# MaxInGaussian/SCFGP

Hardware: AMD Instinct MI355X
Metric: NLML+grad evals/sec (higher is better)
Workload: dtype f32

## Files before the change

### scfgp_amd/csrc/apply.hip

```cpp
#include "kernels.h"
#include "tile_cfgs.h"

#include <algorithm>

#ifdef SCFGP_TRACE
constexpr int ATRACE_CAP = 1 << 16;
__device__ unsigned long long g_atrace[5 * ATRACE_CAP][5];
int64_t apply_trace_read(void* host, int64_t max_bytes) {
    const int64_t n = max_bytes < (int64_t)sizeof(g_atrace) ? max_bytes : (int64_t)sizeof(g_atrace);
    return hipMemcpyFromSymbol(host, HIP_SYMBOL(g_atrace), n) == hipSuccess ? n : -2;
}
#else
int64_t apply_trace_read(void*, int64_t) { return -1; }
#endif
template <typename T, int TILE> struct ApplyCfg {
    typedef TileCfg<T, Tune<T>::APPLY_BM, TILE, SCFGP_BK, Tune<T>::APPLY_WGM, Tune<T>::apply_wgn(TILE), Tune<T>::MS,
                    SCFGP_BK == 16 && Tune<T>::MS == 16> type;
};

#include "apply_epilogue.h"

template <class Cfg, int EPI>
__device__ __forceinline__ void apply_tile(
    const typename Cfg::T* __restrict__ Phi, const typename Cfg::T* __restrict__ Bm, typename Cfg::T* V,
// ... 22 lines not shown
    if constexpr (EPI != 1 && EPI != 4) { if (want_mu) la.dot_reduce(mu + (int64_t)(jt0 + jt) * Np + rb * Cfg::BM); }
    apply_epilogue<Cfg, EPI>(acc, Phi, V, vpart, p, q, y, alpha, ut, K, Kp, Np, rb, cbase, jt0 + jt, smem_raw);
}

template <class Cfg, int EPI>
__global__ __launch_bounds__(Cfg::THREADS) __attribute__((amdgpu_waves_per_eu(1, 8)))
void apply_kernel(
    const typename Cfg::T* __restrict__ Phi, const typename Cfg::T* __restrict__ Bm, typename Cfg::T* V,
    double* __restrict__ vpart, const double* __restrict__ p, const double* __restrict__ q, const double* __restrict__ y,
    const double* __restrict__ alpha, const double* __restrict__ ut, int K, int Kp, int64_t Np, int njt,
    int col0, int jt0, double* __restrict__ mu, int ntot) {
    SMEM_DECL;
    const unsigned wid = xcd_remap(blockIdx.x, gridDim.x);
    if constexpr (EPI == 3 || EPI == 4) {
        const int np = (njt + 1) / 2, t = (int)(wid % np), o = njt - 1 - t;
        const int64_t rb = wid / np;
        apply_tile<Cfg, EPI>(Phi, Bm, V, vpart, p, q, y, alpha, ut, K, Kp, Np, njt, col0, jt0, mu, ntot, t, rb, smem_raw);
        if (o != t) {
            __syncthreads();
            apply_tile<Cfg, EPI>(Phi, Bm, V, vpart, p, q, y, alpha, ut, K, Kp, Np, njt, col0, jt0, mu, ntot, o, rb, smem_raw);
        }
    } else
        apply_tile<Cfg, EPI>(Phi, Bm, V, vpart, p, q, y, alpha, ut, K, Kp, Np, njt, col0, jt0, mu, ntot, (int)(wid % njt), wid / njt, smem_raw);
}

typedef __attribute__((address_space(3))) void lds_void;
typedef const __attribute__((address_space(1))) void gbl_void;
template <typename T, int BN_>
struct ApplyDma {
    static constexpr int ES = (int)sizeof(T), BM = 256, BN = BN_, ROWB = 16 * ES, CPR = ROWB / 16;
    static constexpr int WN = ES == 4 ? 64 : 32;
    static constexpr int WAVES = 4 * (BN / WN), STAGE = (BM + BN) * ROWB, STAGES = 3, LDS_BYTES = STAGES * STAGE,
                         DMA_PER_WAVE = STAGE / 1024 / WAVES, ROWS_PER_DMA = 1024 / ROWB;
    static constexpr int PRE = 2;
    static constexpr int WAVES_PER_EU = WAVES == 4 ? 2 : 4;
    typedef TileCfg<T, BM, BN, 16, 4, BN / WN, 16, true> Cfg;
    static_assert(STAGE / 1024 % WAVES == 0 && LDS_BYTES <= 160 * 1024, "whole DMA instructions per wave; the ring fits the LDS");
    static __device__ __forceinline__ int swz(int x) {
        if constexpr (ES == 4) return (0x78 >> (2 * ((x >> 2) & 3))) & 3;
        else return (int)((0x6BEB08u >> (3 * ((x >> 1) & 7))) & 7);
    }
};
static_assert(((0x6BEB08u >> 0) & 7) == 0 && ((0x6BEB08u >> 3) & 7) == 1 && ((0x6BEB08u >> 6) & 7) == 4 && ((0x6BEB08u >> 9) & 7) == 5 &&
              ((0x6BEB08u >> 12) & 7) == 6 && ((0x6BEB08u >> 15) & 7) == 7 && ((0x6BEB08u >> 18) & 7) == 2 && ((0x6BEB08u >> 21) & 7) == 3,
              "fp64 swizzle table");

template <typename T, int EPI, int BN>
__global__ __launch_bounds__((64 * ApplyDma<T, BN>::WAVES)) __attribute__((amdgpu_waves_per_eu(ApplyDma<T, BN>::WAVES_PER_EU, ApplyDma<T, BN>::WAVES_PER_EU)))
void apply_dma_kernel(const T* __restrict__ Phi, const T* __restrict__ Bm, T* V,
                      double* __restrict__ vpart, const double* __restrict__ p, const double* __restrict__ q,
                      const double* __restrict__ y, const double* __restrict__ alpha, const double* __restrict__ ut,
                      int K, int Kp, int64_t Np, int njt, double* __restrict__ mu, int col0, int slot0, int64_t rb0) {
    typedef ApplyDma<T, BN> D;
    typedef typename D::Cfg Cfg;
    typedef T half_t __attribute__((ext_vector_type(2)));
    typedef std::integral_constant<int, 0> H0;
    typedef std::integral_constant<int, 1> H1;
    constexpr int DPW = D::DMA_PER_WAVE, NRD = Cfg::TM + Cfg::TN, NM = 2 * Cfg::TM * Cfg::TN, PRE = D::PRE;
    static_assert(Cfg::TM == 4 && (Cfg::TN == 4 || Cfg::TN == 2), "fragment lists of the wait statements");
    static_assert(PRE + DPW + NRD <= NM, "one fetch or read per MFMA behind the barrier");
    SMEM_DECL;
    char* smem = smem_raw;
#ifdef SCFGP_TRACE
    const unsigned long long tr_t0 = __builtin_amdgcn_s_memrealtime();
#endif
    const unsigned wid = xcd_remap(blockIdx.x, gridDim.x);
    const int jt = EPI == 3 || EPI == 4 ? (int)((wid % njt + wid / njt) % njt) : (int)(wid % njt);
    const int64_t rb = rb0 + wid / njt;
    const int cbase = col0 + jt * D::BN;
    const int lane = threadIdx.x & 63, wave = __builtin_amdgcn_readfirstlane(threadIdx.x >> 6);
    const char* src[DPW]; unsigned loff[DPW]; int dst[DPW];
#pragma unroll
    for (int u = 0; u < DPW; ++u) {
        const int t = wave * DPW + u, x0 = D::ROWS_PER_DMA * t, l = lane / D::CPR, c = (lane % D::CPR) ^ D::swz(x0 + l);
        const int xb = x0 - D::BM, xcol = (xb & ~(D::WN - 1)) + Cfg::TN * (xb & 15) + ((xb >> 4) & (Cfg::TN - 1));
        const T* rowp = x0 < D::BM ? Phi + (rb * D::BM + x0) * Kp : Bm + (int64_t)(cbase + xcol) * Kp;
        src[u] = reinterpret_cast<const char*>(rowp) + (EPI == 4 ? (cbase / 16) * D::ROWB : 0);
        loff[u] = (unsigned)((x0 < D::BM ? l : Cfg::TN * l) * Kp * D::ES + c * 16);
        dst[u] = t * 1024;
    }
    const auto fetch_one = [&](auto uc, int slot) {
        constexpr int u = decltype(uc)::value;
        __builtin_amdgcn_global_load_lds((gbl_void*)(src[u] + loff[u]), (lds_void*)(smem + slot * D::STAGE + dst[u]), 16, 0, 0);
        src[u] += D::ROWB;
    };
    const int i = lane & 15, qg = lane >> 4;
    const int wm0 = (wave / Cfg::WGN) * Cfg::WM, wn0 = (wave % Cfg::WGN) * Cfg::WN;
    const int hoff0 = sizeof(T) == 4 ? (((qg >> 1) ^ D::swz(i)) << 4) + 8 * (qg & 1) : ((2 * qg) ^ D::swz(i)) << 4;
    const int hoff1 = sizeof(T) == 4 ? (((2 + (qg >> 1)) ^ D::swz(i)) << 4) + 8 * (qg & 1) : ((2 * qg + 1) ^ D::swz(i)) << 4;
    const int ring = (int)(uintptr_t)smem, aoff = ring + (wm0 + i) * D::ROWB, boff = ring + D::BM * D::ROWB + (wn0 + i) * D::ROWB;
    const int ra[2] = {aoff + hoff0, aoff + hoff1}, rbb[2] = {boff + hoff0, boff + hoff1};
    half_t ha[2][Cfg::TM], hb[2][Cfg::TN];
    typename Cfg::MTr::acc_t acc[Cfg::TM][Cfg::TN];
    acc_zero<Cfg>(acc);
    const int nst_all = (K + 15) / 16, nst_tri = (cbase + D::BN + 15) / 16;
    const int nst = (EPI == 3 && nst_tri < nst_all ? nst_tri : nst_all) - (EPI == 4 ? cbase / 16 : 0);
#define SCFGP_LDS_READ(dst, addr, off)                                                                              \
    do {                                                                                                             \
        if constexpr (sizeof(T) == 4) asm volatile("ds_read_b64 %0, %1 offset:%2" : "=v"(dst) : "v"(addr), "n"(off));   \
        else asm volatile("ds_read_b128 %0, %1 offset:%2" : "=v"(dst) : "v"(addr), "n"(off));                           \
    } while (0)
    const auto read_one = [&](auto hc, auto rc, int stage) {
// ... 5 lines not shown
#define SCFGP_WAIT_FRAGS(what, h)                                                                                                   \
    do {                                                                                                                            \
        if constexpr (Cfg::TN == 4)                                                                                                 \
            asm volatile("s_waitcnt " what : "+v"(ha[h][0]), "+v"(ha[h][1]), "+v"(ha[h][2]), "+v"(ha[h][3]),                        \
                                             "+v"(hb[h][0]), "+v"(hb[h][1]), "+v"(hb[h][2]), "+v"(hb[h][3]) :: "memory");           \
        else                                                                                                                        \
            asm volatile("s_waitcnt " what : "+v"(ha[h][0]), "+v"(ha[h][1]), "+v"(ha[h][2]), "+v"(ha[h][3]),                        \
                                             "+v"(hb[h][0]), "+v"(hb[h][1]) :: "memory");                                           \
    } while (0)
    const auto mfma_one = [&](auto hc, auto ic) {
        constexpr int h = decltype(hc)::value, I = decltype(ic)::value, j = I / (Cfg::TM * Cfg::TN), tm = I / Cfg::TN % Cfg::TM, tn = I % Cfg::TN;
        Cfg::MTr::mfma(acc[tm][tn], ha[h][tm][j], hb[h][tn][j]);
        __builtin_amdgcn_sched_barrier(0);
    };
    const auto second_half_pre = [&]() { static_for<PRE>([&](auto ic) { mfma_one(H1(), ic); }); };
    const auto second_half = [&](auto fc, int fslot, int next) {
        static_for<NM - PRE>([&](auto ic) {
            constexpr int I = decltype(ic)::value;
            mfma_one(H1(), std::integral_constant<int, I + PRE>());
            if constexpr (I < DPW) {
                if constexpr (decltype(fc)::value) { fetch_one(ic, fslot); __builtin_amdgcn_sched_barrier(0); }
            } else if constexpr (I - DPW < NRD) {
                read_one(H0(), std::integral_constant<int, I - DPW>(), next);
                __builtin_amdgcn_sched_barrier(0);
            }
        });
    };
    const auto first_half = [&](int next) {
        static_for<NM>([&](auto ic) {
            mfma_one(H0(), ic);
            if constexpr (decltype(ic)::value < NRD) { read_one(H1(), ic, next); __builtin_amdgcn_sched_barrier(0); }
        });
    };
    static_for<DPW>([&](auto uc) { fetch_one(uc, 0); });
    if (nst > 1) static_for<DPW>([&](auto uc) { fetch_one(uc, 1); });
    if (nst > 2) static_for<DPW>([&](auto uc) { fetch_one(uc, 2); });
    if (nst > 2) asm volatile("s_waitcnt vmcnt(%0)" :: "n"(2 * DPW) : "memory");
    else if (nst > 1) asm volatile("s_waitcnt vmcnt(%0)" :: "n"(DPW) : "memory");
    else asm volatile("s_waitcnt vmcnt(0)" ::: "memory");
    __builtin_amdgcn_s_barrier();
    asm volatile("" ::: "memory");
#ifdef SCFGP_TRACE
    const unsigned long long tr_l0 = __builtin_amdgcn_s_memrealtime();
#endif
    static_for<NRD>([&](auto rc) { read_one(H0(), rc, 0); });
    static_for<NRD>([&](auto rc) { read_one(H1(), rc, 0); });
    SCFGP_WAIT_FRAGS("lgkmcnt(0)", 0);
    __builtin_amdgcn_sched_barrier(0);
    static_for<NM>([&](auto ic) { mfma_one(H0(), ic); });
    int slot = 0, s = 0;
    for (; s + 3 < nst; ++s) {
        asm volatile("s_waitcnt vmcnt(%0)" :: "n"(DPW) : "memory");
        SCFGP_WAIT_FRAGS("lgkmcnt(0)", 1);
        __builtin_amdgcn_sched_barrier(0);
        second_half_pre();
        __builtin_amdgcn_s_barrier();
        asm volatile("" ::: "memory");
        const int fslot = slot;
        slot = slot == 2 ? 0 : slot + 1;
        __builtin_amdgcn_sched_barrier(0);
        second_half(std::true_type(), fslot, slot * D::STAGE);
        SCFGP_WAIT_FRAGS("lgkmcnt(0)", 0);
        __builtin_amdgcn_sched_barrier(0);
        first_half(slot * D::STAGE);
    }
    SCFGP_WAIT_FRAGS("lgkmcnt(0)", 1);
    for (; s + 1 < nst; ++s) {
        if (s + 2 < nst) asm volatile("s_waitcnt vmcnt(%0)" :: "n"(DPW) : "memory");
        else asm volatile("s_waitcnt vmcnt(0)" ::: "memory");
        SCFGP_WAIT_FRAGS("lgkmcnt(0)", 1);
        __builtin_amdgcn_sched_barrier(0);
        second_half_pre();
        __builtin_amdgcn_s_barrier();
        asm volatile("" ::: "memory");
        slot = slot == 2 ? 0 : slot + 1;
        __builtin_amdgcn_sched_barrier(0);
        second_half(std::false_type(), 0, slot * D::STAGE);
        SCFGP_WAIT_FRAGS("lgkmcnt(0)", 0);
        __builtin_amdgcn_sched_barrier(0);
        first_half(slot * D::STAGE);
    }
    SCFGP_WAIT_FRAGS("lgkmcnt(0)", 1);
    __builtin_amdgcn_sched_barrier(0);
    static_for<NM>([&](auto ic) { mfma_one(H1(), ic); });
#undef SCFGP_WAIT_FRAGS
    __syncthreads();
#ifdef SCFGP_TRACE
    const unsigned long long tr_l1 = __builtin_amdgcn_s_memrealtime();
#endif
    constexpr int SLOTS = BN >= 128 ? BN / 128 : 1;
    const int vslot = slot0 + SLOTS * jt;
    int tid = (int)threadIdx.x;
    asm volatile("" : "+v"(tid));
    apply_epilogue<Cfg, EPI, EPI == 0 || EPI == 3, true>(acc, Phi, V, vpart, p, q, y, alpha, ut, K, Kp, Np, rb, cbase, vslot, smem_raw, mu, tid);
    if (SLOTS == 2 && (EPI == 0 || EPI == 3) && tid < D::BM) {
        vpart[(int64_t)(vslot + 1) * Np + rb * D::BM + tid] = 0.0;
        if (mu) mu[(int64_t)(vslot + 1) * Np + rb * D::BM + tid] = 0.0;
    }
#ifdef SCFGP_TRACE
    __syncthreads();
    if (threadIdx.x == 0 && blockIdx.x < ATRACE_CAP) {
        unsigned long long* rec = g_atrace[EPI * ATRACE_CAP + blockIdx.x];
        rec[0] = tr_t0; rec[1] = __builtin_amdgcn_s_memrealtime();
        rec[2] = ((unsigned long long)__builtin_amdgcn_s_getreg((20 << 0) | (0 << 6) | (3 << 11)) & 0xF) | ((unsigned long long)jt << 8) |
                                  ((unsigned long long)nst << 20);
        rec[3] = tr_l0; rec[4] = tr_l1;
    }
#endif
}

template <typename T> struct ApplyPlan {
    static constexpr int NW = 2;
    int width[NW], count[NW], col0[NW], jt0[NW], total;
    explicit ApplyPlan(int K) {
        const int w[NW] = {128, 64};
        int col = 0, jt = 0;
        const bool small = K <= 256;
        for (int i = 0; i < NW; ++i) {
            width[i] = w[i];
            const bool last = i == NW - 1;
            count[i] = small && !last ? 0 : (last ? (K - col + w[i] - 1) / w[i] : (K - col) / w[i]);
            col0[i] = col; jt0[i] = jt;
            col += count[i] * w[i]; jt += count[i];
        }
        total = jt;
    }
};
bool F16x3Kernels::apply_runs(const Geom& g) { return ApplyPlan<float>(g.K).count[0] > 0; }
template <class Cfg, int EPI, typename T>
static int apply_launch_cfg(const Geom& g, int njt, int col0, int jt0, const T* Phi, const T* Bm, T* V, double* vpart,
                            const double* p, const double* q, const double* y, const double* alpha, const double* ut,
                            double* mu, int ntot, hipStream_t st) {
    if (njt <= 0) return 0;
    const int64_t nrb = g.Np / Cfg::BM;
    const int wgs_per_rb = EPI == 3 || EPI == 4 ? (njt + 1) / 2 : njt;
    allow_big_lds(apply_kernel<Cfg, EPI>, Cfg::LDS_BYTES);
    hipLaunchKernelGGL((apply_kernel<Cfg, EPI>), dim3((unsigned)(wgs_per_rb * nrb)), dim3(Cfg::THREADS), Cfg::LDS_BYTES, st,
                       Phi, Bm, V, vpart, p, q, y, alpha, ut, g.K, g.Kp, g.Np, njt, col0, jt0, mu, ntot);
    return (int)(njt * nrb);
}
template <typename T, int EPI, int BN>
static int apply_dma_launch(const Geom& g, int njt, int col0, int slot0, const T* Phi, const T* Bm, T* V, double* vpart,
                            const double* p, const double* q, const double* y, const double* alpha, const double* ut,
                            double* mu, hipStream_t st, int64_t rb0 = 0, int64_t nrb = -1) {
    typedef ApplyDma<T, BN> D;
    if (nrb < 0) nrb = g.Np / D::BM;
    if (njt <= 0 || nrb <= 0) return 0;
    allow_big_lds(apply_dma_kernel<T, EPI, BN>, D::LDS_BYTES);
    hipLaunchKernelGGL((apply_dma_kernel<T, EPI, BN>), dim3((unsigned)(njt * nrb)), dim3(64 * D::WAVES), D::LDS_BYTES, st,
                       Phi, Bm, V, vpart, p, q, y, alpha, ut, g.K, g.Kp, g.Np, njt, mu, col0, slot0, rb0);
    return (int)(njt * nrb);
}
static int apply_num_cus() {
    static int n = 0;
    if (n == 0) {
        int dev = 0; hipDeviceProp_t prop;
        if (hipGetDevice(&dev) == hipSuccess && hipGetDeviceProperties(&prop, dev) == hipSuccess) n = prop.multiProcessorCount;
        if (n <= 0) n = 256;
    }
    return n;
}
template <typename T, int EPI>
static int apply_launch(const Geom& g, const T* Phi, const T* Bm, T* V, double* vpart, const double* p, const double* q,
                        const double* y, const double* alpha, const double* ut, double* mu, hipStream_t st,
                        int dma = 0, const T* BmT = nullptr, const F16Operands* f16 = nullptr) {
    if (!BmT) BmT = Bm;
    const ApplyPlan<T> pl(g.K);
    int nb = 0;
    if constexpr (EPI != 2) {
        if (dma && pl.count[0] > 0) {
            int n256 = 0;
            const int64_t nrb = g.Np / 256;
            int64_t tail_rb = 0;
            if constexpr (sizeof(T) == 4) {
                n256 = dma == 2 ? pl.count[0] / 2 : 0;
                if (n256 > 0 && EPI != 3 && EPI != 4) {
                    const int64_t ncu = apply_num_cus(), tiles = nrb * n256, rem = tiles % ncu;
                    if (tiles > ncu && rem > 0 && 20 * rem <= 9 * ncu) tail_rb = (rem + n256 - 1) / n256;
                }
                if (f16 && (EPI == 0 || EPI == 1)) {
                    constexpr int E = EPI == 1 ? 1 : 0;
                    nb += F16x3Kernels::apply<E, 256>(g, n256, 0, 0, Phi, *f16, V, vpart, p, q, y, alpha, ut, mu, st, 0, nrb - tail_rb);
                    nb += F16x3Kernels::apply<E, 128>(g, pl.count[0] - 2 * n256, 256 * n256, 2 * n256, Phi, *f16, V, vpart, p, q, y, alpha, ut, mu, st, 0, nrb - tail_rb);
                    nb += F16x3Kernels::apply<E, 64>(g, pl.count[1], pl.col0[1], pl.jt0[1], Phi, *f16, V, vpart, p, q, y, alpha, ut, mu, st, 0, nrb - tail_rb);
                    if (tail_rb > 0) {
                        nb += F16x3Kernels::apply<E, 128>(g, pl.count[0], 0, 0, Phi, *f16, V, vpart, p, q, y, alpha, ut, mu, st, nrb - tail_rb, tail_rb);
                        nb += F16x3Kernels::apply<E, 64>(g, pl.count[1], pl.col0[1], pl.jt0[1], Phi, *f16, V, vpart, p, q, y, alpha, ut, mu, st, nrb - tail_rb, tail_rb);
                    }
                    return nb;
                }
                nb += apply_dma_launch<T, EPI, 256>(g, n256, 0, 0, Phi, BmT, V, vpart, p, q, y, alpha, ut, mu, st, 0, nrb - tail_rb);
            }
            nb += apply_dma_launch<T, EPI, 128>(g, pl.count[0] - 2 * n256, 256 * n256, 2 * n256, Phi, BmT, V, vpart, p, q, y, alpha, ut, mu, st, 0, nrb - tail_rb);
            nb += apply_dma_launch<T, EPI, 64>(g, pl.count[1], pl.col0[1], pl.jt0[1], Phi, BmT, V, vpart, p, q, y, alpha, ut, mu, st, 0, nrb - tail_rb);
            if (tail_rb > 0) {
                nb += apply_dma_launch<T, EPI, 128>(g, pl.count[0], 0, 0, Phi, BmT, V, vpart, p, q, y, alpha, ut, mu, st, nrb - tail_rb, tail_rb);
                nb += apply_dma_launch<T, EPI, 64>(g, pl.count[1], pl.col0[1], pl.jt0[1], Phi, BmT, V, vpart, p, q, y, alpha, ut, mu, st, nrb - tail_rb, tail_rb);
            }
            return nb;
        }
    }
    nb += apply_launch_cfg<typename ApplyCfg<T, 128>::type, EPI, T>(g, pl.count[0], pl.col0[0], pl.jt0[0], Phi, Bm, V, vpart, p, q, y, alpha, ut, mu, pl.total, st);
    nb += apply_launch_cfg<typename ApplyCfg<T, 64>::type, EPI, T>(g, pl.count[1], pl.col0[1], pl.jt0[1], Phi, Bm, V, vpart, p, q, y, alpha, ut, mu, pl.total, st);
    return nb;
}

template <typename T>
void ApplyKernels<T>::apply_v(const Geom& g, const T* Phi, const T* Bm, T* V, double* vpart, const double* alpha, double* mu,
                              hipStream_t st, int dma, const F16Operands* f16) {
    apply_launch<T, 0>(g, Phi, Bm, V, vpart, nullptr, nullptr, nullptr, alpha, nullptr, mu, st, dma, nullptr, f16);
}
template <typename T>
void ApplyKernels<T>::apply_predict(const Geom& g, const T* Phi, const T* LiT, double* vpart, const double* alpha, double* mu,
                                    hipStream_t st) {
    apply_launch<T, 2>(g, Phi, LiT, (T*)nullptr, vpart, nullptr, nullptr, nullptr, alpha, nullptr, mu, st);
}
template <typename T>
void ApplyKernels<T>::apply_plain(const Geom& g, const T* A, const T* Bm, T* Out, int Kc, int ncols, hipStream_t st) {
    Geom gk = g; gk.K = Kc;
    apply_launch_cfg<typename ApplyCfg<T, 64>::type, 4, T>(gk, (ncols + 63) / 64, 0, 0, A, Bm, Out, nullptr, nullptr, nullptr, nullptr, nullptr,
                                                           nullptr, nullptr, ApplyPlan<T>(Kc).total, st);
}

template <typename T>
void ApplyKernels<T>::apply_c(const Geom& g, const T* Phi, const T* LiT, const T* Li, T* C, double* vpart, const double* alpha,
                              const double* beta, double* mu, hipStream_t st, int dma) {
    const bool by_dma = dma && ApplyPlan<T>(g.K).count[0] > 0;
    apply_launch<T, 3>(g, Phi, LiT, C, vpart, nullptr, nullptr, nullptr, by_dma ? beta : alpha, nullptr, mu, st, dma, Li);
}
template <typename T>
void ApplyKernels<T>::apply_vc(const Geom& g, const T* C, const T* Li, const T* LiT, T* V, hipStream_t st, int dma) {
    apply_launch<T, 4>(g, C, Li, V, nullptr, nullptr, nullptr, nullptr, nullptr, nullptr, nullptr, st, dma, LiT);
}
template <typename T>
void ApplyKernels<T>::apply_phibar(const Geom& g, const T* Phi, const T* Abar, T* V, const double* p, const double* q,
                                   const double* y, const double* alpha, const double* ut, hipStream_t st, int dma, const F16Operands* f16) {
    apply_launch<T, 1>(g, Phi, Abar, V, nullptr, p, q, y, alpha, ut, nullptr, st, dma, nullptr, f16);
}

template <typename T> static int apply_njt(const Geom& g) { return ApplyPlan<T>(g.K).total; }


template <int MODE>
__global__ __launch_bounds__(256) void rowstats_kernel(const double* __restrict__ mupart, const double* __restrict__ vpart, int njt,
                                                       const double* __restrict__ y, const Scal* __restrict__ sc,
                                                       double* __restrict__ o1, double* __restrict__ o2,
                                                       double* __restrict__ partial, int64_t N, int64_t Np) {
    __shared__ double red[4][256];
    const double kappa = sc->kappa;
    double t2 = 0, kb = 0, qv = 0, pm = 0;
    for (int64_t n = (int64_t)blockIdx.x * 256 + threadIdx.x; n < Np; n += (int64_t)gridDim.x * 256) {
        double v = 0, mu = 0;
        for (int t = 0; t < njt; ++t) { v += vpart[(int64_t)t * Np + n]; mu += mupart[(int64_t)t * Np + n]; }
        const double d = kappa * (v + 1.0);
        if (MODE == 0) {
            double pn = 0, qn = 0;
            if (n < N) {
                const double r = mu - y[n];
                const double rv = r * r + v;
                const double e = 1.0 / d - rv / (d * d);
                pn = 2.0 * r / d;
                qn = 1.0 / d + kappa * e;
                t2 += rv / d + log(2.0 * M_PI * d);
                kb += e * (v + 1.0);
                qv += qn * v; pm += pn * mu;
            }
            o1[n] = pn; o2[n] = qn;
        } else if (n < N) {
            o1[n] = mu; o2[n] = sqrt(d);
        }
    }
    if (MODE == 0) {
        red[0][threadIdx.x] = t2; red[1][threadIdx.x] = kb; red[2][threadIdx.x] = qv; red[3][threadIdx.x] = pm;
        __syncthreads();
        for (int w = 128; w >= 1; w >>= 1) {
            if ((int)threadIdx.x < w)
                for (int k = 0; k < 4; ++k) red[k][threadIdx.x] += red[k][threadIdx.x + w];
            __syncthreads();
        }
        if (threadIdx.x < 4) partial[blockIdx.x * 4 + threadIdx.x] = red[threadIdx.x][0];
    }
}

template <typename T>
void ApplyKernels<T>::rowstats(const Geom& g, const double* mupart, const double* vpart, const double* y,
                               const Scal* sc, double* p, double* q, double* partial, int nblocks, hipStream_t st) {
    hipLaunchKernelGGL((rowstats_kernel<0>), dim3(nblocks), dim3(256), 0, st, mupart, vpart, apply_njt<T>(g), y, sc, p, q,
                       partial, g.N, g.Np);
}

template <typename T>
void ApplyKernels<T>::rowpredict(const Geom& g, const double* mupart, const double* vpart, const Scal* sc, double* mu, double* sd,
                                 hipStream_t st) {
    const int nblocks = (int)((g.Np + 255) / 256 < 1024 ? (g.Np + 255) / 256 : 1024);
    hipLaunchKernelGGL((rowstats_kernel<1>), dim3(nblocks), dim3(256), 0, st, mupart, vpart, apply_njt<T>(g),
                       (const double*)nullptr, sc, mu, sd, (double*)nullptr, g.N, g.Np);
}
template <typename T> int ApplyKernels<T>::partials(const Geom& g) { return apply_njt<T>(g); }
__global__ __launch_bounds__(256) void rowresidual_kernel(const double* __restrict__ mupart, int njt, const double* __restrict__ y,
                                                          double* __restrict__ r, int64_t N, int64_t Np) {
    for (int64_t n = (int64_t)blockIdx.x * 256 + threadIdx.x; n < Np; n += (int64_t)gridDim.x * 256) {
        double mu = 0;
        for (int t = 0; t < njt; ++t) mu += mupart[(int64_t)t * Np + n];
        r[n] = n < N ? y[n] - mu : 0.0;
    }
}
template <typename T>
void ApplyKernels<T>::rowresidual(const Geom& g, const double* mupart, const double* y, double* r, hipStream_t st) {
    const int nblocks = (int)((g.Np + 255) / 256 < 1024 ? (g.Np + 255) / 256 : 1024);
    hipLaunchKernelGGL(rowresidual_kernel, dim3(nblocks), dim3(256), 0, st, mupart, apply_njt<T>(g), y, r, g.N, g.Np);
}
template struct ApplyKernels<double>;
template struct ApplyKernels<float>;

__global__ __launch_bounds__(256) void reduce_scalars_kernel(const double* __restrict__ partial, int nblocks, int width,
                                                             double* __restrict__ scalars, int slot0) {
    __shared__ double red[256];
    for (int k = 0; k < width; ++k) {
        double s = 0;
        for (int b = threadIdx.x; b < nblocks; b += 256) s += partial[(int64_t)b * width + k];
        red[threadIdx.x] = s;
        __syncthreads();
        for (int m = 128; m >= 1; m >>= 1) {
            if (threadIdx.x < m) red[threadIdx.x] += red[threadIdx.x + m];
            __syncthreads();
        }
        if (threadIdx.x == 0) scalars[slot0 + k] = red[0];
        __syncthreads();
    }
// ... 54 lines not shown
```

### scfgp_amd/csrc/apply_epilogue.h

```cpp
#pragma once
#include "kernels.h"
#include "tile_cfgs.h"

template <int CTRL> __device__ __forceinline__ double dpp_mov_f64(double x) {
    int lo = __double2loint(x), hi = __double2hiint(x);
    lo = __builtin_amdgcn_update_dpp(0, lo, CTRL, 0xF, 0xF, true);
    hi = __builtin_amdgcn_update_dpp(0, hi, CTRL, 0xF, 0xF, true);
    return __hiloint2double(hi, lo);
}
__device__ __forceinline__ double row16_sum(double x) {
    x += dpp_mov_f64<0xB1>(x);
    x += dpp_mov_f64<0x4E>(x);
    x += dpp_mov_f64<0x141>(x);
    x += dpp_mov_f64<0x140>(x);
    return x;
}
template <class Cfg, int EPI, bool MU>
__device__ __forceinline__ void apply_epilogue_vec2(
    const typename Cfg::MTr::acc_t (&acc)[Cfg::TM][Cfg::TN], const double* __restrict__ Phi, double* V,
    double* __restrict__ vpart, const double* __restrict__ p, const double* __restrict__ q, const double* __restrict__ y,
    const double* __restrict__ alpha, const double* __restrict__ ut, int K, int Kp, int64_t Np, int64_t rb, int cbase, int jtg,
    char* smem_raw, double* __restrict__ mupart, int tid) {
    static_assert(Cfg::TN == 2 && Cfg::MS == 16 && sizeof(typename Cfg::T) == 8 && (EPI == 0 || EPI == 1 || EPI == 3 || EPI == 4), "VEC2 layout");
    AccCoord<Cfg> co(tid);
// ... 46 lines not shown
            if (MU && mupart) mupart[(int64_t)jtg * Np + rb * Cfg::BM + tid] = s2;
        }
    } else {
        double al[2], u2[2];
#pragma unroll
        for (int k = 0; k < 2; ++k) { al[k] = alpha[jg + k]; u2[k] = ut[jg + k]; }
        double* rowsc = reinterpret_cast<double*>(smem_raw);
        for (int i = tid; i < Cfg::BM; i += Cfg::THREADS) {
            const int64_t n = rb * Cfg::BM + i;
            rowsc[3 * i] = 2.0 * q[n]; rowsc[3 * i + 1] = p[n]; rowsc[3 * i + 2] = y[n];
        }
        __syncthreads();
#pragma unroll
        for (int tm = 0; tm < Cfg::TM; ++tm) {
            v2d vv[4];
            int64_t off[4];
#pragma unroll
            for (int r = 0; r < 4; ++r) {
                off[r] = (rb * Cfg::BM + co.row(tm, r)) * Kp + jg;
                vv[r] = *reinterpret_cast<const v2d*>(V + off[r]);
            }
#pragma unroll
            for (int r = 0; r < 4; ++r) {
                const int row = co.row(tm, r);
                const double qn = rowsc[3 * row], pn = rowsc[3 * row + 1], yn = rowsc[3 * row + 2];
                v2d o;
#pragma unroll
                for (int k = 0; k < 2; ++k) o[k] = 2.0 * acc[tm][k][r] + qn * vv[r][k] + pn * al[k] + yn * u2[k];
                *reinterpret_cast<v2d*>(V + off[r]) = o;
            }
        }
    }
}
template <class Cfg, int EPI, bool MU = false, bool VEC4 = false>
__device__ __forceinline__ void apply_epilogue(
    const typename Cfg::MTr::acc_t (&acc)[Cfg::TM][Cfg::TN], const typename Cfg::T* __restrict__ Phi, typename Cfg::T* V,
    double* __restrict__ vpart, const double* __restrict__ p, const double* __restrict__ q, const double* __restrict__ y,
    const double* __restrict__ alpha, const double* __restrict__ ut, int K, int Kp, int64_t Np, int64_t rb, int cbase, int jtg,
    char* smem_raw, double* __restrict__ mupart = nullptr, int tid = (int)threadIdx.x) {
    typedef typename Cfg::T T;
    if constexpr (VEC4 && sizeof(T) == 8) {
        apply_epilogue_vec2<Cfg, EPI, MU>(acc, Phi, V, vpart, p, q, y, alpha, ut, K, Kp, Np, rb, cbase, jtg, smem_raw, mupart, tid);
        return;
    }
    AccCoord<Cfg> co(tid);
    if constexpr (VEC4 && sizeof(T) == 4) {
        static_assert(Cfg::TN == 4 && Cfg::MS == 16 && sizeof(T) == 4 && (EPI == 0 || EPI == 1 || EPI == 3 || EPI == 4), "VEC4 layout");
        const int c4 = co.wn0 + 4 * (co.lane & 15);
        const int jg = cbase + c4;
        if constexpr (EPI == 4) {
#pragma unroll
            for (int tm = 0; tm < Cfg::TM; ++tm)
#pragma unroll
                for (int r = 0; r < 4; ++r)
                    *reinterpret_cast<v4f*>(V + (rb * Cfg::BM + co.row(tm, r)) * Kp + jg) = v4f{acc[tm][0][r], acc[tm][1][r], acc[tm][2][r], acc[tm][3][r]};
        } else if constexpr (EPI == 0 || EPI == 3) {
            double* red = reinterpret_cast<double*>(smem_raw);
            double* red2 = red + Cfg::WGN * Cfg::BM;
            const int wn = (tid >> 6) % Cfg::WGN;
            double al[4], live[4];
#pragma unroll
            for (int k = 0; k < 4; ++k) { live[k] = jg + k < K ? 1.0 : 0.0; al[k] = MU && jg + k < K ? alpha[jg + k] : 0.0; }
#pragma unroll
            for (int tm = 0; tm < Cfg::TM; ++tm) {
                v4f ph[4];
                int64_t off[4];
#pragma unroll
                for (int r = 0; r < 4; ++r) {
                    off[r] = (rb * Cfg::BM + co.row(tm, r)) * Kp + jg;
                    if (EPI == 0) ph[r] = *reinterpret_cast<const v4f*>(Phi + off[r]);
                }
#pragma unroll
                for (int r = 0; r < 4; ++r) {
                    const int row = co.row(tm, r);
                    const v4f c = v4f{acc[tm][0][r], acc[tm][1][r], acc[tm][2][r], acc[tm][3][r]};
                    *reinterpret_cast<v4f*>(V + off[r]) = c;
                    double part = 0, mup = 0;
                    if (EPI == 3) {
                        part = (double)(c[0] * c[0]) + (double)(c[1] * c[1]) + (double)(c[2] * c[2]) + (double)(c[3] * c[3]);
                        if (MU) mup = (double)c[0] * al[0] + (double)c[1] * al[1] + (double)c[2] * al[2] + (double)c[3] * al[3];
                    } else {
#pragma unroll
                        for (int k = 0; k < 4; ++k) { part += (double)ph[r][k] * (double)c[k] * live[k]; if (MU) mup += (double)ph[r][k] * al[k]; }
                    }
                    part = row16_sum(part);
                    if ((co.lane & 15) == 0) red[wn * Cfg::BM + row] = part;
                    if (MU) {
                        mup = row16_sum(mup);
                        if ((co.lane & 15) == 0) red2[wn * Cfg::BM + row] = mup;
                    }
                }
            }
            __syncthreads();
            if (tid < Cfg::BM) {
                double s = 0, s2 = 0;
#pragma unroll
                for (int k = 0; k < Cfg::WGN; ++k) { s += red[k * Cfg::BM + tid]; if (MU) s2 += red2[k * Cfg::BM + tid]; }
                vpart[(int64_t)jtg * Np + rb * Cfg::BM + tid] = s;
                if (MU && mupart) mupart[(int64_t)jtg * Np + rb * Cfg::BM + tid] = s2;
            }
        } else {
            float alf[4], u4f[4];
#pragma unroll
            for (int k = 0; k < 4; ++k) { alf[k] = (float)alpha[jg + k]; u4f[k] = (float)ut[jg + k]; }
            float* rowsc = reinterpret_cast<float*>(smem_raw);
            for (int i = tid; i < Cfg::BM; i += Cfg::THREADS) {
                const int64_t n = rb * Cfg::BM + i;
                rowsc[3 * i] = (float)(2.0 * q[n]); rowsc[3 * i + 1] = (float)p[n]; rowsc[3 * i + 2] = (float)y[n];
            }
            __syncthreads();
#pragma unroll
            for (int tm = 0; tm < Cfg::TM; ++tm) {
                v4f vv[4];
                int64_t off[4];
#pragma unroll
                for (int r = 0; r < 4; ++r) {
                    off[r] = (rb * Cfg::BM + co.row(tm, r)) * Kp + jg;
                    vv[r] = *reinterpret_cast<const v4f*>(V + off[r]);
                }
#pragma unroll
                for (int r = 0; r < 4; ++r) {
                    const int row = co.row(tm, r);
                    const float qn = rowsc[3 * row], pn = rowsc[3 * row + 1], yn = rowsc[3 * row + 2];
                    v4f o;
#pragma unroll
                    for (int k = 0; k < 4; ++k) o[k] = fmaf(qn, vv[r][k], fmaf(pn, alf[k], fmaf(yn, u4f[k], 2.0f * acc[tm][k][r])));
                    *reinterpret_cast<v4f*>(V + off[r]) = o;
                }
            }
        }
        return;
    }
    if (EPI == 4) {
// ... 89 lines not shown
```

### scfgp_amd/csrc/kernels.h

```cpp
#pragma once
#include "common.h"

struct Geom {
    int D, S, M, J, K, P;
    int Dp;
    int Jp;
    int Sp;
    int lowrank;
    int Kp;
    int tile;
    int gfull;
    int gstrip;
    int64_t N;
    int64_t Np;
};

struct RowSplits {
    int nsplit;
    int groups;
    int units;
    int taper;
    int gran;
    int64_t nrb;
    __host__ __device__ int per_group() const { return units + taper; }
// ... 22 lines not shown
    static void featuremap(const Geom& g, const double* Xt, const Projection& pr, const Scal* sc, T* Phi, hipStream_t st);
    static void convert(const double* src, T* dst, int K, int Kp, hipStream_t st);
    static void convert_transposed(const double* src, T* dst, int K, int Kp, hipStream_t st);
};

template <typename T>
struct GramKernels {
    static void gram(const Geom& g, const T* Phi, const double* w, const double* side, const RowSplits& rs, int64_t chunk,
                     double* slabs, double* sidepart, int* qhead, float* ws2, hipStream_t st);
    static int gram_jobs(const Geom& g);
    static void xtz(const Geom& g, const double* Xt, const T* Phi, const T* Phibar, int nsplit, int64_t chunk, double* slabs,
                    hipStream_t st);
    static void zbar_inplace(const Geom& g, const T* Phi, T* Phibar, hipStream_t st);
    static void rsel(const Geom& g, const double* params, T* out, hipStream_t st);
    static void tn_plain(const double* A, int Dp, const T* Bm, int64_t ldb, int J, int64_t Np, int nsplit, int64_t chunk, double* slabs,
                         hipStream_t st);
};

struct F16Operands { const unsigned* Phi16; const char* B16; const float* scale; unsigned* V16; const float* vbound; };

template <typename T>
struct ApplyKernels {
    static void apply_v(const Geom& g, const T* Phi, const T* Bm, T* V, double* vpart, const double* alpha, double* mupart,
                        hipStream_t st, int dma = 0, const F16Operands* f16 = nullptr);
    static void apply_predict(const Geom& g, const T* Phi, const T* LiT, double* vpart, const double* alpha, double* mupart,
                              hipStream_t st);
    static void apply_c(const Geom& g, const T* Phi, const T* LiT, const T* Li, T* C, double* vpart, const double* alpha,
                        const double* beta, double* mupart, hipStream_t st, int dma = 0);
    static void apply_vc(const Geom& g, const T* C, const T* Li, const T* LiT, T* V, hipStream_t st, int dma = 0);
    static void apply_phibar(const Geom& g, const T* Phi, const T* Abar, T* V, const double* p, const double* q,
                             const double* y, const double* alpha, const double* ut, hipStream_t st, int dma = 0, const F16Operands* f16 = nullptr);
    static void apply_plain(const Geom& g, const T* A, const T* Bm, T* Out, int Kc, int ncols, hipStream_t st);
    static void rowstats(const Geom& g, const double* mupart, const double* vpart, const double* y,
                         const Scal* sc, double* p, double* q, double* partial, int nblocks, hipStream_t st);
    static void rowpredict(const Geom& g, const double* mupart, const double* vpart, const Scal* sc, double* mu, double* sd,
                           hipStream_t st);
    static void rowresidual(const Geom& g, const double* mupart, const double* y, double* r, hipStream_t st);
    static int partials(const Geom& g);
};

struct F16x3Kernels {
    static void split_operand(const Geom& g, const double* M, char* B16, float* scale, double* part, const Scal* sc, hipStream_t st);
    template <int EPI, int BN>
    static int apply(const Geom& g, int njt, int col0, int slot0, const float* Phi, const F16Operands& f, float* V,
                     double* vpart, const double* p, const double* q, const double* y, const double* alpha, const double* ut, double* mu,
                     hipStream_t st, int64_t rb0, int64_t nrb);
    static bool apply_runs(const Geom& g);
    static constexpr size_t F16_PAD = 1024;
    static int side_blocks(const Geom& g);
    static void split_phi(const Geom& g, const float* Phi, const double* y, const Scal* sc, unsigned* Phi16, double* sidepart, float* tmp,
                          hipStream_t st);
    static void v_bound(const Geom& g, const double* B, const Scal* sc, float* tmp, hipStream_t st);
    static void split_v(const Geom& g, const float* V, const double* q, const double* p, unsigned* V16g, unsigned* qV16g, double* sidepart,
                        float* tmp, hipStream_t st);
    static int gram_chunks(const Geom& g, int64_t chunk);
    static int gram_tiles(const Geom& g);
    static void gram(const Geom& g, const unsigned* A16g, const unsigned* B16g, const float* scale, int64_t chunk, double* slabs, hipStream_t st);
};

template <typename T> struct SweepKernels : FmapKernels<T>, GramKernels<T>, ApplyKernels<T> {};

int64_t trace_read(void* host, int64_t max_bytes);
int64_t apply_trace_read(void* host, int64_t max_bytes);
int64_t chol_trace_read(void* host, int64_t max_bytes);

void reduce_tri_tiles(const double* slabs, int nsplit, int nts, int tile, double* packed, hipStream_t st);
void unpack_tri_tiles(const double* packed, int nts, int tile, double* full, int64_t ld, hipStream_t st);
// ... 145 lines not shown
```

### scfgp_amd/csrc/scfgp_api.hip

```cpp
#include "../../include/scfgp_hip.h"
#include "kernels.h"

#include <dlfcn.h>
#if __has_include(<rccl/rccl.h>)
#include <rccl/rccl.h>
#else
extern "C" {
typedef struct ncclComm* ncclComm_t;
typedef struct { char internal[128]; } ncclUniqueId;
typedef enum { ncclSuccess = 0 } ncclResult_t;
typedef enum { ncclFloat64 = 8 } ncclDataType_t;
typedef enum { ncclSum = 0 } ncclRedOp_t;
ncclResult_t ncclGetUniqueId(ncclUniqueId*);
ncclResult_t ncclCommInitRank(ncclComm_t*, int, ncclUniqueId, int);
ncclResult_t ncclAllReduce(const void*, void*, size_t, ncclDataType_t, ncclRedOp_t, ncclComm_t, hipStream_t);
ncclResult_t ncclCommDestroy(ncclComm_t);
const char* ncclGetErrorString(ncclResult_t);
}
#endif

#include <algorithm>
#include <cmath>
#include <cstdlib>
#include <cstring>
// ... 497 lines not shown
        const Geom& g = c->g;
        { ProfScope ps(c, "kstage_factor");
          hipMemcpyAsync(c->d_x1 + (int64_t)g.Kp * g.Kp, c->d_xp1 + c->n_pk, sizeof(double) * (g.Kp + 8), hipMemcpyDeviceToDevice, c->st);
          kstage_factor(c->kstage(), c->d_xp1, c->d_sc, c->st); }
        if (c->last_cform) {
            SK::convert(c->d_Li, (T*)c->d_BT, g.K, g.Kp, c->st);
            SK::convert_transposed(c->d_Li, (T*)c->d_AbarT, g.K, g.Kp, c->st);
        } else {
            SK::convert(c->d_B, (T*)c->d_BT, g.K, g.Kp, c->st);
            if (c->f16_on()) {
                F16x3Kernels::split_operand(g, c->d_B, c->d_B16, c->d_f16scale, c->d_partial, c->d_sc, c->st);
                F16x3Kernels::v_bound(g, c->d_B, c->d_sc, c->d_f16tmp, c->st);
            }
        }
        HIPCHK(c, hipGetLastError());
        return SCFGP_OK;
    }
    static int pass2(scfgp_ctx* c, int want_grad) {
        const Geom& g = c->g;
        if (c->last_cform) {
            const int dma = c->dma() ? 1 : 0;
            { ProfScope ps(c, "apply_c");
              SK::apply_c(g, (const T*)c->d_Phi, (const T*)c->d_AbarT, (const T*)c->d_BT, (T*)c->d_C, c->d_vpart, c->alpha(), c->beta(), c->d_mu, c->st, dma); }
            { ProfScope ps(c, "apply_vc");
              SK::apply_vc(g, (const T*)c->d_C, (const T*)c->d_BT, (const T*)c->d_AbarT, (T*)c->d_V, c->st, dma); }
        } else {
            ProfScope ps(c, "apply_v");
            F16Operands f16 = c->f16ops();
            if (want_grad && c->f16_gram()) f16.V16 = c->d_V16g;
            SK::apply_v(g, (const T*)c->d_Phi, (const T*)c->d_BT, (T*)c->d_V, c->d_vpart, c->alpha(), c->d_mu, c->st, c->dma(), c->f16_on() ? &f16 : nullptr);
        }
        const int nb = (int)std::min<int64_t>(g.Np / 4, 2048);
        { ProfScope ps(c, "rowstats");
          SK::rowstats(g, c->d_mu, c->d_vpart, c->d_y, c->d_sc, c->d_p, c->d_q, c->d_partial, nb, c->st);
          reduce_scalars(c->d_partial, nb, 4, c->xs2(), 0, c->st);
          write_status(c->xs2(), 0.0, 0.0, 0.0, 0.0, c->st); }
        if (want_grad) {
            gram_to(c, c->last_cform ? (const T*)c->d_C : (const T*)c->d_V, c->d_q, c->d_p, c->d_xp2, "gram_w");
        }
        HIPCHK(c, hipGetLastError());
        return SCFGP_OK;
    }
    static int adjoint(scfgp_ctx* c) {
        const Geom& g = c->g;
        { ProfScope ps(c, "kstage_adjoint"); unpack_exchange(c, c->d_xp2, c->d_x2);
          if (c->last_cform) kstage_adjoint_factor_form(c->kstage(), c->d_x2, c->d_Abar, c->d_sc, c->st);
          else kstage_adjoint(c->kstage(), c->d_x2, c->d_Abar, c->d_sc, c->st);
          kstage_bbar(c->kstage(), c->d_xp1, c->d_Abar, c->d_partial, c->st); }
        SK::convert(c->d_Abar, (T*)c->d_AbarT, g.K, g.Kp, c->st);
        if (c->f16_on()) F16x3Kernels::split_operand(g, c->d_Abar, c->d_B16, c->d_f16scale, c->d_partial, c->d_sc, c->st);
        HIPCHK(c, hipGetLastError());
        return SCFGP_OK;
    }
    static int pass3(scfgp_ctx* c) {
        const Geom& g = c->g;
        { ProfScope ps(c, "apply_phibar");
          const F16Operands f16 = c->f16ops();
          SK::apply_phibar(g, (const T*)c->d_Phi, (const T*)c->d_AbarT, (T*)c->d_V, c->d_p, c->d_q, c->d_y, c->alpha(), c->ut(), c->st, c->dma(),
                           c->f16_on() ? &f16 : nullptr);
          write_status(c->x3_scalars(), 0.0, 0.0, 0.0, 0.0, c->st); }
        const int ntm = c->Dpp / XT, ntn = g.Jp / XT;
        const int64_t chunk = c->dtype == SCFGP_F32 ? c->gram_chunk : 0;
        c->last_lrb = c->want_lrb();
        if (c->last_lrb) {
            ProfScope ps(c, "xtz");
            T* Zb = (T*)c->d_V; T* U = (T*)c->d_V + g.Jp;
            SK::zbar_inplace(g, (const T*)c->d_Phi, Zb, c->st);
// ... 2198 lines not shown
```

Baseline: 4.900.

## Fold tail row-blocks into the BN=64 launch and stage epilogue scalars via LDS DMA

The tail row-blocks, which were previously run as two extra kernel launches (BN=128 and BN=64), are now handled as edge workgroups appended to the BN=64 DMA launch. That launch now covers the narrow columns for every row block, and rowstats sums a different number of partial slots for the edge rows. The EPI==1 fp32 path also prefetches q, p, y, alpha and ut into extra LDS with global_load_lds before the main loop, so the epilogue reads scalars from LDS rather than global memory. The aim is fewer launches, less tail imbalance and lower epilogue latency, at the cost of more LDS per workgroup and more complex slot indexing.

Result: no change. 4.921 (median of 6 runs) (+0.4%).

```diff
diff --git a/scfgp_amd/csrc/apply.hip b/scfgp_amd/csrc/apply.hip
--- a/scfgp_amd/csrc/apply.hip
+++ b/scfgp_amd/csrc/apply.hip
@@ -78,6 +78,9 @@
     static constexpr int WN = ES == 4 ? 64 : 32;
     static constexpr int WAVES = 4 * (BN / WN), STAGE = (BM + BN) * ROWB, STAGES = 3, LDS_BYTES = STAGES * STAGE,
                          DMA_PER_WAVE = STAGE / 1024 / WAVES, ROWS_PER_DMA = 1024 / ROWB;
+    static constexpr bool SCALARS = ES == 4 && BN != 128;
+    static constexpr int SC_ROW_DMA = BM * 8 / 1024, SC_COL_DMA = (BN * 8 + 1023) / 1024, SC_DMA = 3 * SC_ROW_DMA + 2 * SC_COL_DMA,
+                         SC_BYTES = SC_DMA * 1024;
     static constexpr int PRE = 2;
     static constexpr int WAVES_PER_EU = WAVES == 4 ? 2 : 4;
     typedef TileCfg<T, BM, BN, 16, 4, BN / WN, 16, true> Cfg;
@@ -96,7 +99,8 @@
 void apply_dma_kernel(const T* __restrict__ Phi, const T* __restrict__ Bm, T* V,
                       double* __restrict__ vpart, const double* __restrict__ p, const double* __restrict__ q,
                       const double* __restrict__ y, const double* __restrict__ alpha, const double* __restrict__ ut,
-                      int K, int Kp, int64_t Np, int njt, double* __restrict__ mu, int col0, int slot0, int64_t rb0) {
+                      int K, int Kp, int64_t Np, int njt, double* __restrict__ mu, int col0, int slot0, int64_t rb0,
+                      unsigned wg_main, int64_t rb1) {
     typedef ApplyDma<T, BN> D;
     typedef typename D::Cfg Cfg;
     typedef T half_t __attribute__((ext_vector_type(2)));
@@ -111,9 +115,22 @@
     const unsigned long long tr_t0 = __builtin_amdgcn_s_memrealtime();
 #endif
     const unsigned wid = xcd_remap(blockIdx.x, gridDim.x);
-    const int jt = EPI == 3 || EPI == 4 ? (int)((wid % njt + wid / njt) % njt) : (int)(wid % njt);
-    const int64_t rb = rb0 + wid / njt;
-    const int cbase = col0 + jt * D::BN;
+    constexpr bool EDGE = BN == 64 && sizeof(T) == 4 && (EPI == 0 || EPI == 1);
+    constexpr int SLOTS = BN >= 128 ? BN / 128 : 1;
+    int jt, cbase, vslot;
+    int64_t rb;
+    if (!EDGE || wid < wg_main) {
+        jt = EPI == 3 || EPI == 4 ? (int)((wid % njt + wid / njt) % njt) : (int)(wid % njt);
+        rb = rb0 + wid / njt;
+        cbase = col0 + jt * D::BN;
+        vslot = slot0 + SLOTS * jt;
+    } else {
+        const unsigned w = wid - wg_main, npc = (unsigned)(col0 / D::BN);
+        jt = (int)(w % npc);
+        rb = rb1 + w / npc;
+        cbase = jt * D::BN;
+        vslot = (jt & 1) ? slot0 + njt + (jt >> 1) : jt >> 1;
+    }
     const int lane = threadIdx.x & 63, wave = __builtin_amdgcn_readfirstlane(threadIdx.x >> 6);
     const char* src[DPW]; unsigned loff[DPW]; int dst[DPW];
 #pragma unroll
@@ -185,6 +202,21 @@
             if constexpr (decltype(ic)::value < NRD) { read_one(H1(), ic, next); __builtin_amdgcn_sched_barrier(0); }
         });
     };
+    constexpr bool SCAL = D::SCALARS && EPI == 1;
+    if constexpr (SCAL) {
+        static_for<D::SC_DMA>([&](auto tc) {
+            constexpr int t = decltype(tc)::value, c = t - 3 * D::SC_ROW_DMA;
+            if (wave == t % D::WAVES) {
+                const double* s;
+                if constexpr (c < 0) s = (t < D::SC_ROW_DMA ? q : t < 2 * D::SC_ROW_DMA ? p : y) + rb * D::BM + (t % D::SC_ROW_DMA) * 128 + 2 * lane;
+                else {
+                    const int cl = 128 * (c % D::SC_COL_DMA) + 2 * lane;
+                    s = (c < D::SC_COL_DMA ? alpha : ut) + cbase + (cl < D::BN - 2 ? cl : D::BN - 2);
+                }
+                __builtin_amdgcn_global_load_lds((gbl_void*)s, (lds_void*)(smem + D::LDS_BYTES + t * 1024), 16, 0, 0);
+            }
+        });
+    }
     static_for<DPW>([&](auto uc) { fetch_one(uc, 0); });
     if (nst > 1) static_for<DPW>([&](auto uc) { fetch_one(uc, 1); });
     if (nst > 2) static_for<DPW>([&](auto uc) { fetch_one(uc, 2); });
@@ -241,11 +273,9 @@
 #ifdef SCFGP_TRACE
     const unsigned long long tr_l1 = __builtin_amdgcn_s_memrealtime();
 #endif
-    constexpr int SLOTS = BN >= 128 ? BN / 128 : 1;
-    const int vslot = slot0 + SLOTS * jt;
     int tid = (int)threadIdx.x;
     asm volatile("" : "+v"(tid));
-    apply_epilogue<Cfg, EPI, EPI == 0 || EPI == 3, true>(acc, Phi, V, vpart, p, q, y, alpha, ut, K, Kp, Np, rb, cbase, vslot, smem_raw, mu, tid);
+    apply_epilogue<Cfg, EPI, EPI == 0 || EPI == 3, true, SCAL ? D::LDS_BYTES : -1>(acc, Phi, V, vpart, p, q, y, alpha, ut, K, Kp, Np, rb, cbase, vslot, smem_raw, mu, tid);
     if (SLOTS == 2 && (EPI == 0 || EPI == 3) && tid < D::BM) {
         vpart[(int64_t)(vslot + 1) * Np + rb * D::BM + tid] = 0.0;
         if (mu) mu[(int64_t)(vslot + 1) * Np + rb * D::BM + tid] = 0.0;
@@ -295,14 +325,19 @@
 template <typename T, int EPI, int BN>
 static int apply_dma_launch(const Geom& g, int njt, int col0, int slot0, const T* Phi, const T* Bm, T* V, double* vpart,
                             const double* p, const double* q, const double* y, const double* alpha, const double* ut,
-                            double* mu, hipStream_t st, int64_t rb0 = 0, int64_t nrb = -1) {
+                            double* mu, hipStream_t st, int64_t rb0 = 0, int64_t nrb = -1, int64_t edge_rb = 0) {
     typedef ApplyDma<T, BN> D;
     if (nrb < 0) nrb = g.Np / D::BM;
-    if (njt <= 0 || nrb <= 0) return 0;
-    allow_big_lds(apply_dma_kernel<T, EPI, BN>, D::LDS_BYTES);
-    hipLaunchKernelGGL((apply_dma_kernel<T, EPI, BN>), dim3((unsigned)(njt * nrb)), dim3(64 * D::WAVES), D::LDS_BYTES, st,
-                       Phi, Bm, V, vpart, p, q, y, alpha, ut, g.K, g.Kp, g.Np, njt, mu, col0, slot0, rb0);
-    return (int)(njt * nrb);
+    if (njt < 0 || nrb <= 0) return 0;
+    const int64_t main = (int64_t)njt * nrb, edge = edge_rb * (col0 / BN);
+    if (main + edge <= 0) return 0;
+    constexpr int lds = D::LDS_BYTES + (D::SCALARS && EPI == 1 ? D::SC_BYTES : 0);
+    static_assert(lds == D::LDS_BYTES || lds * (D::WAVES == 16 ? 1 : 2) <= 160 * 1024, "with the scalars, as many workgroups per CU as without");
+    allow_big_lds(apply_dma_kernel<T, EPI, BN>, lds);
+    hipLaunchKernelGGL((apply_dma_kernel<T, EPI, BN>), dim3((unsigned)(main + edge)), dim3(64 * D::WAVES), lds, st,
+                       Phi, Bm, V, vpart, p, q, y, alpha, ut, g.K, g.Kp, g.Np, njt, mu, col0, slot0, rb0, (unsigned)main,
+                       rb0 + nrb - edge_rb);
+    return (int)(main + edge);
 }
 static int apply_num_cus() {
     static int n = 0;
@@ -312,6 +347,15 @@
         if (n <= 0) n = 256;
     }
     return n;
+}
+static int64_t apply_tail_rb(int64_t nrb, int n256) {
+    if (n256 <= 0) return 0;
+    const int64_t ncu = apply_num_cus(), tiles = nrb * n256, rem = tiles % ncu;
+    return tiles > ncu && rem > 0 && 20 * rem <= 9 * ncu ? (rem + n256 - 1) / n256 : 0;
+}
+template <typename T> static int64_t apply_edge_rb(const Geom& g, int dma, bool f16) {
+    if (sizeof(T) != 4 || dma != 2 || f16) return 0;
+    return apply_tail_rb(g.Np / 256, ApplyPlan<T>(g.K).count[0] / 2);
 }
 template <typename T, int EPI>
 static int apply_launch(const Geom& g, const T* Phi, const T* Bm, T* V, double* vpart, const double* p, const double* q,
@@ -327,10 +371,7 @@
             int64_t tail_rb = 0;
             if constexpr (sizeof(T) == 4) {
                 n256 = dma == 2 ? pl.count[0] / 2 : 0;
-                if (n256 > 0 && EPI != 3 && EPI != 4) {
-                    const int64_t ncu = apply_num_cus(), tiles = nrb * n256, rem = tiles % ncu;
-                    if (tiles > ncu && rem > 0 && 20 * rem <= 9 * ncu) tail_rb = (rem + n256 - 1) / n256;
-                }
+                if (EPI != 3 && EPI != 4) tail_rb = apply_tail_rb(nrb, n256);
                 if (f16 && (EPI == 0 || EPI == 1)) {
                     constexpr int E = EPI == 1 ? 1 : 0;
                     nb += F16x3Kernels::apply<E, 256>(g, n256, 0, 0, Phi, *f16, V, vpart, p, q, y, alpha, ut, mu, st, 0, nrb - tail_rb);
@@ -345,11 +386,7 @@
                 nb += apply_dma_launch<T, EPI, 256>(g, n256, 0, 0, Phi, BmT, V, vpart, p, q, y, alpha, ut, mu, st, 0, nrb - tail_rb);
             }
             nb += apply_dma_launch<T, EPI, 128>(g, pl.count[0] - 2 * n256, 256 * n256, 2 * n256, Phi, BmT, V, vpart, p, q, y, alpha, ut, mu, st, 0, nrb - tail_rb);
-            nb += apply_dma_launch<T, EPI, 64>(g, pl.count[1], pl.col0[1], pl.jt0[1], Phi, BmT, V, vpart, p, q, y, alpha, ut, mu, st, 0, nrb - tail_rb);
-            if (tail_rb > 0) {
-                nb += apply_dma_launch<T, EPI, 128>(g, pl.count[0], 0, 0, Phi, BmT, V, vpart, p, q, y, alpha, ut, mu, st, nrb - tail_rb, tail_rb);
-                nb += apply_dma_launch<T, EPI, 64>(g, pl.count[1], pl.col0[1], pl.jt0[1], Phi, BmT, V, vpart, p, q, y, alpha, ut, mu, st, nrb - tail_rb, tail_rb);
-            }
+            nb += apply_dma_launch<T, EPI, 64>(g, pl.count[1], pl.col0[1], pl.jt0[1], Phi, BmT, V, vpart, p, q, y, alpha, ut, mu, st, 0, nrb, tail_rb);
             return nb;
         }
     }
@@ -398,13 +435,15 @@
 __global__ __launch_bounds__(256) void rowstats_kernel(const double* __restrict__ mupart, const double* __restrict__ vpart, int njt,
                                                        const double* __restrict__ y, const Scal* __restrict__ sc,
                                                        double* __restrict__ o1, double* __restrict__ o2,
-                                                       double* __restrict__ partial, int64_t N, int64_t Np) {
+                                                       double* __restrict__ partial, int64_t N, int64_t Np,
+                                                       int njt_edge, int64_t edge_row0) {
     __shared__ double red[4][256];
     const double kappa = sc->kappa;
     double t2 = 0, kb = 0, qv = 0, pm = 0;
     for (int64_t n = (int64_t)blockIdx.x * 256 + threadIdx.x; n < Np; n += (int64_t)gridDim.x * 256) {
         double v = 0, mu = 0;
-        for (int t = 0; t < njt; ++t) { v += vpart[(int64_t)t * Np + n]; mu += mupart[(int64_t)t * Np + n]; }
+        const int nt = n >= edge_row0 ? njt_edge : njt;
+        for (int t = 0; t < nt; ++t) { v += vpart[(int64_t)t * Np + n]; mu += mupart[(int64_t)t * Np + n]; }
         const double d = kappa * (v + 1.0);
         if (MODE == 0) {
             double pn = 0, qn = 0;
@@ -437,9 +476,11 @@
 
 template <typename T>
 void ApplyKernels<T>::rowstats(const Geom& g, const double* mupart, const double* vpart, const double* y,
-                               const Scal* sc, double* p, double* q, double* partial, int nblocks, hipStream_t st) {
-    hipLaunchKernelGGL((rowstats_kernel<0>), dim3(nblocks), dim3(256), 0, st, mupart, vpart, apply_njt<T>(g), y, sc, p, q,
-                       partial, g.N, g.Np);
+                               const Scal* sc, double* p, double* q, double* partial, int nblocks, hipStream_t st, int dma, bool f16) {
+    const int njt = apply_njt<T>(g);
+    const int64_t edge_rb = apply_edge_rb<T>(g, dma, f16);
+    hipLaunchKernelGGL((rowstats_kernel<0>), dim3(nblocks), dim3(256), 0, st, mupart, vpart, njt, y, sc, p, q,
+                       partial, g.N, g.Np, njt + ApplyPlan<T>(g.K).count[0], g.Np - 256 * edge_rb);
 }
 
 template <typename T>
@@ -447,7 +488,7 @@
                                  hipStream_t st) {
     const int nblocks = (int)((g.Np + 255) / 256 < 1024 ? (g.Np + 255) / 256 : 1024);
     hipLaunchKernelGGL((rowstats_kernel<1>), dim3(nblocks), dim3(256), 0, st, mupart, vpart, apply_njt<T>(g),
-                       (const double*)nullptr, sc, mu, sd, (double*)nullptr, g.N, g.Np);
+                       (const double*)nullptr, sc, mu, sd, (double*)nullptr, g.N, g.Np, 0, g.Np);
 }
 template <typename T> int ApplyKernels<T>::partials(const Geom& g) { return apply_njt<T>(g); }
 __global__ __launch_bounds__(256) void rowresidual_kernel(const double* __restrict__ mupart, int njt, const double* __restrict__ y,
diff --git a/scfgp_amd/csrc/apply_epilogue.h b/scfgp_amd/csrc/apply_epilogue.h
--- a/scfgp_amd/csrc/apply_epilogue.h
+++ b/scfgp_amd/csrc/apply_epilogue.h
@@ -102,7 +102,7 @@
         }
     }
 }
-template <class Cfg, int EPI, bool MU = false, bool VEC4 = false>
+template <class Cfg, int EPI, bool MU = false, bool VEC4 = false, int SCOFF = -1>
 __device__ __forceinline__ void apply_epilogue(
     const typename Cfg::MTr::acc_t (&acc)[Cfg::TM][Cfg::TN], const typename Cfg::T* __restrict__ Phi, typename Cfg::T* V,
     double* __restrict__ vpart, const double* __restrict__ p, const double* __restrict__ q, const double* __restrict__ y,
@@ -169,6 +169,42 @@
                 vpart[(int64_t)jtg * Np + rb * Cfg::BM + tid] = s;
                 if (MU && mupart) mupart[(int64_t)jtg * Np + rb * Cfg::BM + tid] = s2;
             }
+        } else if constexpr (SCOFF >= 0) {
+            const double* sc = reinterpret_cast<const double*>(smem_raw + SCOFF);
+            const double *qd = sc, *pd = sc + Cfg::BM, *yd = sc + 2 * Cfg::BM, *ald = sc + 3 * Cfg::BM, *utd = ald + (Cfg::BN + 127) / 128 * 128;
+            float alf[4], u4f[4];
+#pragma unroll
+            for (int k = 0; k < 4; ++k) { alf[k] = (float)ald[c4 + k]; u4f[k] = (float)utd[c4 + k]; }
+            const int wm0 = (__builtin_amdgcn_readfirstlane(tid >> 6) / Cfg::WGN) * Cfg::WM;
+            typedef __attribute__((address_space(1))) char gchar;
+            typedef __attribute__((address_space(1))) v4f gv4f;
+            gchar* const vrows = (gchar*)(V + (rb * Cfg::BM + wm0) * Kp);
+            const unsigned lo = (unsigned)((co.row(0, 0) - co.wm0) * Kp + jg) * 4u;
+#pragma unroll
+            for (int tb = 0; tb < Cfg::TM; tb += 2) {
+                v4f vv[2][4];
+                gchar* rowp[2][4];
+#pragma unroll
+                for (int h = 0; h < 2; ++h)
+#pragma unroll
+                    for (int r = 0; r < 4; ++r) {
+                        rowp[h][r] = vrows + (int64_t)((tb + h) * Cfg::MS + r) * Kp * 4;
+                        asm volatile("" : "+s"(rowp[h][r]));
+                        vv[h][r] = *(const gv4f*)(rowp[h][r] + lo);
+                    }
+                __builtin_amdgcn_sched_barrier(0);
+#pragma unroll
+                for (int h = 0; h < 2; ++h)
+#pragma unroll
+                    for (int r = 0; r < 4; ++r) {
+                        const int row = co.row(tb + h, r);
+                        const float qn = (float)(2.0 * qd[row]), pn = (float)pd[row], yn = (float)yd[row];
+                        v4f o;
+#pragma unroll
+                        for (int k = 0; k < 4; ++k) o[k] = fmaf(qn, vv[h][r][k], fmaf(pn, alf[k], fmaf(yn, u4f[k], 2.0f * acc[tb + h][k][r])));
+                        *(gv4f*)(rowp[h][r] + lo) = o;
+                    }
+            }
         } else {
             float alf[4], u4f[4];
 #pragma unroll
diff --git a/scfgp_amd/csrc/kernels.h b/scfgp_amd/csrc/kernels.h
--- a/scfgp_amd/csrc/kernels.h
+++ b/scfgp_amd/csrc/kernels.h
@@ -78,7 +78,7 @@
                              const double* y, const double* alpha, const double* ut, hipStream_t st, int dma = 0, const F16Operands* f16 = nullptr);
     static void apply_plain(const Geom& g, const T* A, const T* Bm, T* Out, int Kc, int ncols, hipStream_t st);
     static void rowstats(const Geom& g, const double* mupart, const double* vpart, const double* y,
-                         const Scal* sc, double* p, double* q, double* partial, int nblocks, hipStream_t st);
+                         const Scal* sc, double* p, double* q, double* partial, int nblocks, hipStream_t st, int dma = 0, bool f16 = false);
     static void rowpredict(const Geom& g, const double* mupart, const double* vpart, const Scal* sc, double* mu, double* sd,
                            hipStream_t st);
     static void rowresidual(const Geom& g, const double* mupart, const double* y, double* r, hipStream_t st);
diff --git a/scfgp_amd/csrc/scfgp_api.hip b/scfgp_amd/csrc/scfgp_api.hip
--- a/scfgp_amd/csrc/scfgp_api.hip
+++ b/scfgp_amd/csrc/scfgp_api.hip
@@ -553,7 +553,7 @@
         }
         const int nb = (int)std::min<int64_t>(g.Np / 4, 2048);
         { ProfScope ps(c, "rowstats");
-          SK::rowstats(g, c->d_mu, c->d_vpart, c->d_y, c->d_sc, c->d_p, c->d_q, c->d_partial, nb, c->st);
+          SK::rowstats(g, c->d_mu, c->d_vpart, c->d_y, c->d_sc, c->d_p, c->d_q, c->d_partial, nb, c->st, c->last_cform ? 0 : c->dma(), c->f16_on());
           reduce_scalars(c->d_partial, nb, 4, c->xs2(), 0, c->st);
           write_status(c->xs2(), 0.0, 0.0, 0.0, 0.0, c->st); }
         if (want_grad) {
```
